# zubair-irshad/articulated-object-nerf

Hardware: AMD Instinct MI355X
Metric: rays/sec (64c+128f samples) (higher is better)
Workload: dtype f32; 1 GPU; sapien-single-scene vanilla NeRF full-frame render 640x480, 65 coarse + 193 fine evals/ray, 307200 rays per GPU per step, randomized=False, white_bkgd=True; rays_per_gpu=307200, evals_per_ray=258, exchange=none

## Files before the change

### articulated-object-nerf_amd/csrc/aon_common.h

```cpp
#pragma once

#include <hip/hip_runtime.h>
#include <stdint.h>

#include <atomic>

namespace aon {

typedef float f32x4 __attribute__((ext_vector_type(4)));
typedef float f32x16 __attribute__((ext_vector_type(16)));

#define AON_HALF_PI_F32 1.57079637050628662109375f

__device__ __forceinline__ float sin_f32(float x) {
  const float ax = __builtin_fabsf(x);
  const float k = __builtin_rintf(ax * 0.636619747f);
  const int q = (int)k;
  float r = __builtin_fmaf(k, -0x1.921fb4p+0f, ax);
  r = __builtin_fmaf(k, -0x1.4442d0p-24f, r);
  r = __builtin_fmaf(k, -0x1.846988p-48f, r);
  const float z = r * r;
  float ps = __builtin_fmaf(z, -1.9515295891e-4f, 8.3321608736e-3f);
  ps = __builtin_fmaf(z, ps, -1.6666654611e-1f);
  const float s = __builtin_fmaf(r * z, ps, r);
  float pc = __builtin_fmaf(z, 2.443315711809948e-5f, -1.388731625493765e-3f);
  pc = __builtin_fmaf(z, pc, 4.166664568298827e-2f);
  const float c = __builtin_fmaf(z * z, pc, __builtin_fmaf(z, -0.5f, 1.0f));
  float res = (q & 1) ? c : s;
  res = (q & 2) ? -res : res;
  return x < 0.f ? -res : res;
}

__device__ __forceinline__ float cos_f32(float x) {
  const float ax = __builtin_fabsf(x);
  const float k = __builtin_rintf(ax * 0.636619747f);
  const int q = (int)k;
  float r = __builtin_fmaf(k, -0x1.921fb4p+0f, ax);
  r = __builtin_fmaf(k, -0x1.4442d0p-24f, r);
  r = __builtin_fmaf(k, -0x1.846988p-48f, r);
  const float z = r * r;
  float ps = __builtin_fmaf(z, -1.9515295891e-4f, 8.3321608736e-3f);
  ps = __builtin_fmaf(z, ps, -1.6666654611e-1f);
  const float s = __builtin_fmaf(r * z, ps, r);
  float pc = __builtin_fmaf(z, 2.443315711809948e-5f, -1.388731625493765e-3f);
  pc = __builtin_fmaf(z, pc, 4.166664568298827e-2f);
  const float c = __builtin_fmaf(z * z, pc, __builtin_fmaf(z, -0.5f, 1.0f));
  float res = (q & 1) ? s : c;
  return ((q + 1) & 2) ? -res : res;
}

__device__ __forceinline__ float softplus_f32(float x) {
  const float z = __builtin_amdgcn_exp2f(__fmul_rn(__builtin_fabsf(x), -1.44269502162933349609375f));
  float p = 0.001986696617677808f;
  p = __builtin_fmaf(p, z, -0.013187826611101627f);
  p = __builtin_fmaf(p, z, 0.041006576269865036f);
  p = __builtin_fmaf(p, z, -0.08188041299581528f);
  p = __builtin_fmaf(p, z, 0.12377995997667313f);
  p = __builtin_fmaf(p, z, -0.16087622940540314f);
  p = __builtin_fmaf(p, z, 0.19885820150375366f);
  p = __builtin_fmaf(p, z, -0.24986496567726135f);
  p = __builtin_fmaf(p, z, 0.33332496881484985f);
  p = __builtin_fmaf(p, z, -0.4999997913837433f);
  p = __builtin_fmaf(p, z, 1.0f);
  return __fadd_rn(__builtin_fmaxf(x, 0.f), __fmul_rn(z, p));
}

__device__ __forceinline__ float sigmoid_f32(float x) {
  const float e = __builtin_amdgcn_exp2f(__fmul_rn(x, -1.44269502162933349609375f));
  const float d = __fadd_rn(1.0f, e);
  const float r = __builtin_amdgcn_rcpf(d);
  const float s = __builtin_fmaf(__builtin_fmaf(-d, r, 1.0f), r, r);
  return x < -87.0f ? 0.f : s;
}

__device__ __forceinline__ float torch_max(float a, float b) {
  if (a != a || b != b) return __builtin_nanf("");
  return a < b ? b : a;
}
__device__ __forceinline__ float torch_min(float a, float b) {
  if (a != a || b != b) return __builtin_nanf("");
  return b < a ? b : a;
}

constexpr int kNetWidth = 256;
constexpr int kCondWidth = 128;
constexpr int kPosEnc = 63;
constexpr int kViewEnc = 27;

constexpr int kChL0 = 0;
constexpr int kChL1 = 2;
constexpr int kChL5 = 34;
constexpr int kChL6 = 44;
constexpr int kChL7 = 52;
constexpr int kChBott = 60;
constexpr int kChView = 68;
constexpr int kNumChunks = 77;
constexpr int kNumBigChunks = 68;
constexpr int kBigChunkBytes = 8 * 4096;
constexpr int kSmallChunkBytes = 4 * 4096;

__host__ __device__ constexpr int chunk_bytes(int c) { return c < kNumBigChunks ? kBigChunkBytes : kSmallChunkBytes; }
__host__ __device__ constexpr int64_t chunk_offset(int c) {
  return c < kNumBigChunks ? (int64_t)c * kBigChunkBytes
                           : (int64_t)kNumBigChunks * kBigChunkBytes + (int64_t)(c - kNumBigChunks) * kSmallChunkBytes;
}
constexpr int64_t kStreamBytes = chunk_offset(kNumChunks);

constexpr int kChFView = 60;
constexpr int kNumChunksF = 69;
__host__ __device__ constexpr int chunk_bytes_f(int c) { return c < kChFView ? kBigChunkBytes : kSmallChunkBytes; }
__host__ __device__ constexpr int64_t chunk_offset_f(int c) {
  return c < kChFView ? (int64_t)c * kBigChunkBytes : (int64_t)kChFView * kBigChunkBytes + (int64_t)(c - kChFView) * kSmallChunkBytes;
}
constexpr int64_t kStreamBytesF = chunk_offset_f(kNumChunksF);
constexpr int64_t kFoldTmpOff = kStreamBytesF;
static_assert(kStreamBytesF + (128 * 256 + 128) * 4 <= kStreamBytes, "fold temporaries fit between the folded stream and the small block");

constexpr int kSmBias = 0;
constexpr int kSmBiasBott = 8 * 256;
constexpr int kSmBiasView = kSmBiasBott + 256;
constexpr int kSmWSigma = kSmBiasView + 128;
constexpr int kSmWRgb = kSmWSigma + 256;
constexpr int kSmBSigma = kSmWRgb + 384;
constexpr int kSmBRgb = kSmBSigma + 1;
constexpr int kSmallFloats = 3076;
constexpr int64_t kSmallBytes = kSmallFloats * 4;

constexpr int64_t kPackedBytes = kStreamBytes + kSmallBytes;

constexpr int kPlE = 0;
__host__ __device__ constexpr int plane_h(int l) { return 64 + 256 * l; }
constexpr int kPlBot = 64 + 8 * 256;
constexpr int kPlVE = kPlBot + 256;
constexpr int kPlHV = kPlVE + 32;
constexpr int kPlRows = kPlHV + 128;
constexpr int kMaskLayers = 9;

constexpr int kAPlPos = 0;
__host__ __device__ constexpr int aplane_d(int l) { return 32 + 128 * l; }
constexpr int kAPlE = 32 + 4 * 128;
__host__ __device__ constexpr int aplane_h(int l) { return kAPlE + 64 + 256 * l; }
constexpr int kAPlBot = kAPlE + 64 + 8 * 256;
constexpr int kAPlVE = kAPlBot + 256;
__host__ __device__ constexpr int aplane_v(int l) { return kAPlVE + 32 + 128 * l; }
constexpr int kAPlRows = kAPlVE + 32 + 4 * 128;
constexpr int kAMaskLayers = 16;

constexpr int kNumVanillaParams = 24;

struct ActParams {
  int act;
  float rgb_scale, rgb_shift, sigma_bias;
  const float* noise;
  float noise_std;
};
inline ActParams default_act(int act) { return ActParams{act, 1.002f, 0.001f, -1.0f, nullptr, 0.f}; }

struct ChainSeg {
  const char* packed_bwd;
  const float* small;
  const float* d_raw;
  const void* masks;
  const float* planes;
  float* dplanes;
  float* dxp;
  int64_t Np;
};

struct TrainSeg {
  const char* packed;
  const float* small;
  const float* rays_o; const float* rays_d; const float* viewdirs;
  const float* t_vals;
  int64_t n_rays; int S;
  float* raw;
  float* planes; void* masks;
  int64_t np_total;
  const float* view_bias = nullptr;
};

template <class T>
__device__ __forceinline__ T block_excl_scan(T v, T& total, T* red) {
  constexpr int kThreads = 256;
  const int lane = threadIdx.x & 63, wave = threadIdx.x >> 6;
  T x = v;
#pragma unroll
  for (int d = 1; d < 64; d <<= 1) {
    const T y = __shfl_up(x, d);
    if (lane >= d) x += y;
  }
  if (lane == 63) red[wave] = x;
  __syncthreads();
  T base = 0;
  total = 0;
#pragma unroll
  for (int w = 0; w < kThreads / 64; ++w) {
    const T t = red[w];
    if (w < wave) base += t;
    total += t;
  }
  __syncthreads();
  return base + x - v;
}

struct OccGrid {
  const uint32_t* bits;
  int64_t cells[3];
  float lo[3], step[3], hi[3];
};

constexpr int kMaxDevices = 64;

struct DeviceOnce {
  std::atomic<uint64_t> done{0};
};

template <class Kernel>
inline hipError_t set_max_lds(Kernel* kernel, int bytes, DeviceOnce& once) {
  int dev = 0;
  if (hipError_t e = hipGetDevice(&dev); e != hipSuccess) return e;
  if (dev < 0 || dev >= kMaxDevices) return hipErrorInvalidDevice;
  const uint64_t bit = 1ull << dev;
  if (once.done.load(std::memory_order_acquire) & bit) return hipSuccess;
  if (hipError_t e = hipFuncSetAttribute(reinterpret_cast<const void*>(kernel), hipFuncAttributeMaxDynamicSharedMemorySize, bytes);
      e != hipSuccess)
    return e;
  once.done.fetch_or(bit, std::memory_order_release);
  return hipSuccess;
}

}
```

### articulated-object-nerf_amd/csrc/aon_mlp.hip

```cpp
#include "aon_launch.h"
#include "aon_mlp_core.h"

namespace aon {

struct VanillaNet {
  static constexpr int kSlotBytes = kPairSlotBytes;
  static constexpr bool kPair = true;
  static constexpr int kNumChunks = aon::kNumChunks;
  static constexpr int chunk_bytes(int c) { return aon::chunk_bytes(c); }
};
struct VanillaFoldNet {
  static constexpr int kSlotBytes = kPairSlotBytes;
  static constexpr bool kPair = true;
  static constexpr int kNumChunks = aon::kNumChunksF;
  static constexpr int chunk_bytes(int c) { return aon::chunk_bytes_f(c); }
};
struct VanillaFoldVbNet {
  static constexpr int kSlotBytes = kPairSlotBytes;
  static constexpr bool kPair = true;
  static constexpr int kNumChunks = aon::kNumChunksF - 1;
  static constexpr int chunk_bytes(int c) { return aon::chunk_bytes_f(c < kChFView ? c : c + 1); }
  static constexpr int skip_before(int c) { return c == kChFView ? kSmallChunkBytes : 0; }
};

struct PackArgs {
  const float* p[kNumVanillaParams];
};

template <bool FOLD>
__global__ void pack_vanilla_kernel(PackArgs a, float* __restrict__ packed, int L, int Lv) {
  const int P = 3 + 6 * L, V = 3 + 6 * Lv;
  const int64_t idx = (int64_t)blockIdx.x * blockDim.x + threadIdx.x;
  constexpr int64_t stream_floats = kStreamBytes / 4;
  constexpr int64_t used_floats = FOLD ? kStreamBytesF / 4 : stream_floats;
  const float* Wf = packed + kFoldTmpOff / 4;
  if (idx >= stream_floats + kSmallFloats) return;
  if (idx >= used_floats && idx < stream_floats) {
    if (idx >= used_floats + 128 * 256 + 128) packed[idx] = 0.f;
    return;
  }
  if (idx >= stream_floats) {
    const int s = (int)(idx - stream_floats);
    float v = 0.f;
    if (s < kSmBiasBott) v = a.p[2 * (s >> 8) + 1][s & 255];
    else if (s < kSmBiasView) v = a.p[19][s - kSmBiasBott];
    else if (s < kSmWSigma) v = FOLD ? Wf[128 * 256 + s - kSmBiasView] : a.p[17][s - kSmBiasView];
    else if (s < kSmWRgb) v = a.p[20][s - kSmWSigma];
    else if (s < kSmBSigma) v = a.p[22][s - kSmWRgb];
    else if (s < kSmBRgb) v = a.p[21][0];
    else if (s < kSmBRgb + 3) v = a.p[23][s - kSmBRgb];
    packed[idx] = v;
    return;
  }
  int c, r, nt;
  constexpr int nbig = FOLD ? kChFView : kNumBigChunks;
  if (idx < (int64_t)nbig * (kBigChunkBytes / 4)) {
    c = (int)(idx / (kBigChunkBytes / 4)); r = (int)(idx % (kBigChunkBytes / 4)); nt = 8;
  } else {
    const int64_t i2 = idx - (int64_t)nbig * (kBigChunkBytes / 4);
    c = nbig + (int)(i2 / (kSmallChunkBytes / 4)); r = (int)(i2 % (kSmallChunkBytes / 4)); nt = 4;
    if constexpr (FOLD) c = c == kChFView ? kChView + 8 : c - 1 + (kChView - kChFView);
  }
  const int cc = r & 3, lane = (r >> 2) & 63, rest = r >> 8;
  const int tp = rest % nt, q = rest / nt;
  const int h = lane >> 5, row = 32 * tp + (lane & 31);
  const float* W; int ld, n_out = 256, col;
  const int hid_col = 8 * q + 4 * h + cc;
  auto pcol = [&](int c63) { return c63 < 0 ? -1 : pos_col_in(c63, L); };
  auto vcol = [&](int c27) { return c27 < 0 ? -1 : view_col_in(c27, Lv); };
  if (c < kChL1) { W = a.p[0]; ld = P; col = pcol(posenc_col(c, q, cc, h)); }
  else if (c < kChL5) { const int l = 1 + (c - kChL1) / 8; W = a.p[2 * l]; ld = 256; col = 32 * ((c - kChL1) % 8) + hid_col; }
  else if (c < kChL5 + 8) { W = a.p[10]; ld = 256 + P; col = 32 * (c - kChL5) + hid_col; }
  else if (c < kChL6) { W = a.p[10]; ld = 256 + P; col = pcol(posenc_col(c - kChL5 - 8, q, cc, h)); if (col >= 0) col += 256; }
  else if (c < kChL7) { W = a.p[12]; ld = 256; col = 32 * (c - kChL6) + hid_col; }
  else if (c < kChBott) { W = a.p[14]; ld = 256; col = 32 * (c - kChL7) + hid_col; }
  else if (c < kChView) { W = a.p[18]; ld = 256; col = 32 * (c - kChBott) + hid_col; }
  else if (c < kChView + 8) {
    W = a.p[16]; ld = 256 + V; n_out = kCondWidth; col = 32 * (c - kChView) + hid_col;
    if constexpr (FOLD) { W = Wf; ld = 256; }
  }
  else { W = a.p[16]; ld = 256 + V; n_out = kCondWidth; col = vcol(viewenc_col(q, cc, h)); if (col >= 0) col += 256; }
  packed[idx] = (col >= 0 && row < n_out) ? W[(int64_t)row * ld + col] : 0.f;
}

struct MlpSeg {
  const char* packed;
  const float* rays_o;
  const float* rays_d;
  const float* viewdirs;
  const float* t_vals;
  const float* samples_enc;
  const float* viewdirs_enc;
  float* raw;
  int64_t total;
  int S;
  int npass;
  union {
    float* planes;
    const int* gather_idx;
  };
  union {
    u32x4* masks;
    const int64_t* gather_count;
  };
  int64_t Np;
  const float* view_bias;
};
struct MlpArgs {
  MlpSeg seg[2];
  int npass_total;
};

constexpr int kLdsBytes = kRingBytes + (int)kSmallBytes;

template <bool ENC_IN_KERNEL, bool TRAIN, bool FOLD, bool VB = false, bool GATHER = false>
__global__ void __launch_bounds__(256) mlp_fwd_kernel(MlpArgs args) {
  static_assert(FOLD || !VB, "the per-ray view bias belongs to the folded form");
  static_assert(!GATHER || (ENC_IN_KERNEL && !TRAIN), "the occupancy list serves the inference kernel on in-kernel encodings");
  using Net = std::conditional_t<VB, VanillaFoldVbNet, std::conditional_t<FOLD, VanillaFoldNet, VanillaNet>>;
  extern __shared__ __attribute__((aligned(16))) char smem[];
  float* sm = reinterpret_cast<float*>(smem + kRingBytes);

  const int tid = threadIdx.x;
  const int lane = tid & 63, wave = tid >> 6;
  const int m = lane & 31, h = lane >> 5;
  const int wave_s = __builtin_amdgcn_readfirstlane(wave);

  const int64_t listed = GATHER ? *args.seg[0].gather_count : 0;
  const int npass0 = GATHER ? (int)((listed + 127) / 128) : args.seg[0].npass;
  int cur = (int)blockIdx.x >= npass0 ? 1 : 0;
  auto load_small = [&](const char* packed) {
    const f32x4* src = reinterpret_cast<const f32x4*>(packed + kStreamBytes);
    f32x4* dst = reinterpret_cast<f32x4*>(sm);
    for (int i = tid; i < kSmallFloats / 4; i += 256) dst[i] = src[i];
  };
  load_small(args.seg[cur].packed);

  Pipe p;
  pipe_init<Net>(p, args.seg[cur].packed, smem, wave, lane);

  for (int gpass = blockIdx.x; gpass < (GATHER ? npass0 : args.npass_total); gpass += gridDim.x) {
    const int si = gpass >= npass0 ? 1 : 0;
    if (si != cur) {
      __syncthreads();
      load_small(args.seg[si].packed);
      __syncthreads();
      cur = si;
    }
    const MlpSeg& sg = args.seg[si];
    const int pass = gpass - (si ? npass0 : 0);
    {
      const int nxt = gpass + (int)gridDim.x;
      p.stream = sg.packed;
      p.next_stream = args.seg[(nxt >= npass0 && nxt < (GATHER ? npass0 : args.npass_total)) ? 1 : si].packed;
    }
    int64_t g = (int64_t)pass * 128 + wave * 32 + m;
    bool valid;
    int64_t gc;
    if constexpr (GATHER) {
      valid = g < listed;
      g = gc = sg.gather_idx[valid ? g : listed - 1];
    } else {
      valid = g < sg.total;
      gc = valid ? g : sg.total - 1;
    }
    const int64_t ray = gc / sg.S;

    f32x16 E[2], V;
    float x[3] = {0.f, 0.f, 0.f}, vd[3] = {0.f, 0.f, 0.f};
    if constexpr (ENC_IN_KERNEL) {
      const float t = sg.t_vals[gc];
#pragma unroll
      for (int a = 0; a < 3; ++a) {
        x[a] = __fadd_rn(sg.rays_o[ray * 3 + a], __fmul_rn(t, sg.rays_d[ray * 3 + a]));
        vd[a] = sg.viewdirs[ray * 3 + a];
      }
      encode_pos(x, h, E);
      if constexpr (!VB || TRAIN) encode_view(vd, h, V);
    } else {
      load_pos_enc(sg.samples_enc + gc * kPosEnc, h, E);
      if constexpr (!VB || TRAIN) load_view_enc(sg.viewdirs_enc + ray * kViewEnc, h, V);
    }
    int ray32 = (int)ray;
    (void)ray32;

    PlaneIO io{};
    unsigned moff = 0;
    if constexpr (TRAIN) { io = make_plane_io(sg.planes, kPlRows, (int64_t)pass * 4 + wave_s, m, h); moff = mask_lane_off(pass, tid); }
    if constexpr (TRAIN) {
      store_pos_enc_plane(E, io, kPlE, h);
      store_view_enc_plane(V, io, kPlVE, h);
    }
    auto consume = [&](const f32x16 (&in)[8], int in_row, u32x4& mw, bool with_mask) {
      return [&, in_row, with_mask](int j) {
        return [&, in_row, with_mask, j](int i) {
          if constexpr (TRAIN) {
            if (i < 16) {
              if ((i & 3) == 0) store_quad<false>(io, in_row + 32 * j, i >> 2, in[j]);
              if (with_mask) mw[j >> 1] = mask_push_post(mw[j >> 1], in[j][i]);
            }
          }
        };
      };
    };
    auto put_mask = [&](const u32x4& mw, int mask_layer) {
      if constexpr (TRAIN)
        *mask_ptr(sg.masks, sg.Np, mask_layer, moff) = u32x4{mask_word_finish(mw[0]), mask_word_finish(mw[1]), mask_word_finish(mw[2]), mask_word_finish(mw[3])};
    };
    f32x16 X[8], Y[8];
    u32x4 mw;
    init_bias(X, sm + kSmBias + 0 * 256, h);
    chunk_mma<Net, kChL0 + 0, 8, 16>(p, E[0], X);
    chunk_mma<Net, kChL0 + 1, 8, 16>(p, E[1], X);
    relu_tiles(X);
    mw = u32x4{0u, 0u, 0u, 0u}; init_bias(Y, sm + kSmBias + 1 * 256, h); dense_layer<Net, kChL1 + 0, 8, 8>(p, X, Y, consume(X, plane_h(0), mw, true)); put_mask(mw, 0); relu_tiles(Y);
    mw = u32x4{0u, 0u, 0u, 0u}; init_bias(X, sm + kSmBias + 2 * 256, h); dense_layer<Net, kChL1 + 8, 8, 8>(p, Y, X, consume(Y, plane_h(1), mw, true)); put_mask(mw, 1); relu_tiles(X);
    mw = u32x4{0u, 0u, 0u, 0u}; init_bias(Y, sm + kSmBias + 3 * 256, h); dense_layer<Net, kChL1 + 16, 8, 8>(p, X, Y, consume(X, plane_h(2), mw, true)); put_mask(mw, 2); relu_tiles(Y);
    mw = u32x4{0u, 0u, 0u, 0u}; init_bias(X, sm + kSmBias + 4 * 256, h); dense_layer<Net, kChL1 + 24, 8, 8>(p, Y, X, consume(Y, plane_h(3), mw, true)); put_mask(mw, 3); relu_tiles(X);
    mw = u32x4{0u, 0u, 0u, 0u}; init_bias(Y, sm + kSmBias + 5 * 256, h);
    dense_layer<Net, kChL5, 8, 8>(p, X, Y, consume(X, plane_h(4), mw, true)); put_mask(mw, 4);
#ifdef AON_TRAIN_REENCODE
    if constexpr (TRAIN && ENC_IN_KERNEL) {
      asm volatile("" : "+v"(x[0]), "+v"(x[1]), "+v"(x[2]));
      encode_pos(x, h, E);
    }
#endif
    if constexpr (TRAIN && !ENC_IN_KERNEL) {
      int64_t gq = gc;
      asm volatile("" : "+v"(gq));
      load_pos_enc(sg.samples_enc + gq * kPosEnc, h, E);
    }
    chunk_mma<Net, kChL5 + 8, 8, 16>(p, E[0], Y);
    chunk_mma<Net, kChL5 + 9, 8, 16>(p, E[1], Y);
    relu_tiles(Y);
    mw = u32x4{0u, 0u, 0u, 0u}; init_bias(X, sm + kSmBias + 6 * 256, h); dense_layer<Net, kChL6, 8, 8>(p, Y, X, consume(Y, plane_h(5), mw, true)); put_mask(mw, 5); relu_tiles(X);
    f32x16 Z[4];
    mw = u32x4{0u, 0u, 0u, 0u}; init_bias(Y, sm + kSmBias + 7 * 256, h);
    if constexpr (VB) {
      asm volatile("" : "+v"(ray32));
      const float* vb = sg.view_bias + (int64_t)ray32 * kCondWidth + 4 * h;
      auto l7_side = [&](int j) {
        auto base = consume(X, plane_h(6), mw, true)(j);
        return [&, base, j, vb](int i) {
          base(i);
          if (j == 7 && i < 16) {
            const f32x4 v = *reinterpret_cast<const f32x4*>(vb + 32 * (i >> 2) + 8 * (i & 3));
            Z[i >> 2][4 * (i & 3)] = v[0]; Z[i >> 2][4 * (i & 3) + 1] = v[1]; Z[i >> 2][4 * (i & 3) + 2] = v[2]; Z[i >> 2][4 * (i & 3) + 3] = v[3];
          }
        };
      };
      dense_layer<Net, kChL7, 8, 8>(p, X, Y, l7_side);
    } else {
      dense_layer<Net, kChL7, 8, 8>(p, X, Y, consume(X, plane_h(6), mw, true));
    }
    put_mask(mw, 6); relu_tiles(Y);
    float sigma = head_partial<8>(Y, sm + kSmWSigma, h);
    sigma = sigma + __shfl_xor(sigma, 32) + sm[kSmBSigma];
    constexpr int kChV = FOLD ? kChFView : kChView;
    auto reencode_view = [&]() {
      if constexpr (TRAIN && ENC_IN_KERNEL) {
        asm volatile("" : "+v"(vd[0]), "+v"(vd[1]), "+v"(vd[2]));
        encode_view(vd, h, V);
      }
      if constexpr (TRAIN && !ENC_IN_KERNEL) {
        int64_t rq = ray;
        asm volatile("" : "+v"(rq));
        load_view_enc(sg.viewdirs_enc + rq * kViewEnc, h, V);
      }
    };
    if constexpr (FOLD) {
      mw = u32x4{0u, 0u, 0u, 0u};
      if constexpr (!VB) {
        init_bias(Z, sm + kSmBiasView, h);
        reencode_view();
        chunk_mma<Net, kChV, 4, 14>(p, V, Z);
      }
      dense_layer<Net, kChV + (VB ? 0 : 1), 8, 4>(p, Y, Z, consume(Y, plane_h(7), mw, true)); put_mask(mw, 7);
    } else {
      mw = u32x4{0u, 0u, 0u, 0u}; init_bias(X, sm + kSmBiasBott, h); dense_layer<Net, kChBott, 8, 8>(p, Y, X, consume(Y, plane_h(7), mw, true)); put_mask(mw, 7);
      init_bias(Z, sm + kSmBiasView, h);
      dense_layer<Net, kChV, 8, 4>(p, X, Z, consume(X, kPlBot, mw, false));
      reencode_view();
      chunk_mma<Net, kChV + 8, 4, 14>(p, V, Z);
    }
    relu_tiles(Z);
    if constexpr (TRAIN) {
      *mask_ptr(sg.masks, sg.Np, 8, moff) = relu_mask_bits(Z);
      store_plane(Z, io, kPlHV);
    }
    float rgb[3];
#pragma unroll
    for (int ch = 0; ch < 3; ++ch) {
      float v = head_partial<4>(Z, sm + kSmWRgb + ch * kCondWidth, h);
      rgb[ch] = v + __shfl_xor(v, 32) + sm[kSmBRgb + ch];
    }
    if (valid && h == 0) {
      f32x4 o; o[0] = rgb[0]; o[1] = rgb[1]; o[2] = rgb[2]; o[3] = sigma;
      reinterpret_cast<f32x4*>(sg.raw)[g] = o;
    }
  }
  asm volatile("s_waitcnt vmcnt(0)" ::: "memory");
}

void vanilla_fold_jobs_fwd(const float* const* params, float* packed, int view_levels, FoldGemm jobs[2]) {
  float* Wf = packed + kFoldTmpOff / 4;
  fold_view_jobs(params[16], 256 + 3 + 6 * view_levels, params[17], params[18], params[19], Wf, Wf + 128 * 256, jobs);
}

hipError_t launch_pack_vanilla(const float* const* params, float* packed, hipStream_t stream, int pos_levels, int view_levels, bool fold_done) {
  PackArgs a;
  for (int i = 0; i < kNumVanillaParams; ++i) a.p[i] = params[i];
  const int64_t n = kStreamBytes / 4 + kSmallFloats;
  const int form = fold_default();
  set_stream_form(packed, form);
  if (form == kFormFolded) {
    if (!fold_done) {
      FoldGemm jobs[2];
      vanilla_fold_jobs_fwd(params, packed, view_levels, jobs);
      if (hipError_t e = launch_fold_gemms(jobs, 2, stream); e != hipSuccess) return e;
    }
    pack_vanilla_kernel<true><<<dim3((unsigned)((n + 255) / 256)), dim3(256), 0, stream>>>(a, packed, pos_levels, view_levels);
  } else {
    pack_vanilla_kernel<false><<<dim3((unsigned)((n + 255) / 256)), dim3(256), 0, stream>>>(a, packed, pos_levels, view_levels);
  }
  return hipGetLastError();
}

int num_cus() {
  static std::atomic<int> cache[kMaxDevices];
  int dev = 0;
  if (hipGetDevice(&dev) != hipSuccess) return -1;
  if (dev < 0 || dev >= kMaxDevices) return -1;
  int cus = cache[dev].load(std::memory_order_relaxed);
  if (cus == 0) {
    hipDeviceProp_t prop;
    if (hipGetDeviceProperties(&prop, dev) != hipSuccess) return -1;
    cus = prop.multiProcessorCount;
    cache[dev].store(cus, std::memory_order_relaxed);
  }
  return cus;
}

template <bool ENC, bool TRAIN, bool FOLD, bool VB = false, bool GATHER = false>
static hipError_t launch_mlp_tf(const MlpArgs& args, hipStream_t stream) {
  static DeviceOnce lds_once;
  if (hipError_t e = set_max_lds(&mlp_fwd_kernel<ENC, TRAIN, FOLD, VB, GATHER>, kLdsBytes, lds_once); e != hipSuccess) return e;
  const int g_num_cus = num_cus();
  if (g_num_cus <= 0) return hipErrorInvalidDevice;
  const int grid = args.npass_total < g_num_cus ? args.npass_total : g_num_cus;
  if (grid <= 0) return hipSuccess;
  mlp_fwd_kernel<ENC, TRAIN, FOLD, VB, GATHER><<<dim3(grid), dim3(256), kLdsBytes, stream>>>(args);
  return hipGetLastError();
}

template <bool ENC, bool TRAIN, bool GATHER = false>
static hipError_t launch_mlp_t(const MlpArgs& args, hipStream_t stream) {
  const int form = stream_form(args.seg[0].packed);
  if (form == kFormUnknown) return hipErrorInvalidValue;
  if (args.seg[1].npass > 0 && stream_form(args.seg[1].packed) != form) return hipErrorInvalidValue;
  const bool vb = args.seg[0].view_bias != nullptr;
  if (args.seg[1].npass > 0 && (args.seg[1].view_bias != nullptr) != vb) return hipErrorInvalidValue;
  if (vb && form != kFormFolded) return hipErrorInvalidValue;
  if constexpr (ENC) {
    if (vb) return launch_mlp_tf<ENC, TRAIN, true, true, GATHER>(args, stream);
  } else {
    if (vb) return hipErrorInvalidValue;
  }
  return form == kFormFolded ? launch_mlp_tf<ENC, TRAIN, true, false, GATHER>(args, stream)
                             : launch_mlp_tf<ENC, TRAIN, false, false, GATHER>(args, stream);
}

__global__ __launch_bounds__(256) void view_bias_kernel(const float* chunk, const float* bias_vec, const float* viewdirs, int64_t n_rays, float* out) {
  __shared__ float enc[8][2][16];
  const int tid = threadIdx.x;
  const int64_t ray0 = (int64_t)blockIdx.x * 8;
  if (tid < 16) {
    const int64_t ray = ray0 + (tid >> 1);
    if (ray < n_rays) {
      float vd[3] = {viewdirs[ray * 3], viewdirs[ray * 3 + 1], viewdirs[ray * 3 + 2]};
      f32x16 V;
      encode_view(vd, tid & 1, V);
#pragma unroll
      for (int r = 0; r < 16; ++r) enc[tid >> 1][tid & 1][r] = V[r];
    }
  }
  const int row = tid & 127, tp = row >> 5;
  const float bias = bias_vec[row];
  float w[14][2];
#pragma unroll
  for (int r = 0; r < 14; ++r)
#pragma unroll
    for (int hh = 0; hh < 2; ++hh) w[r][hh] = chunk[((((r >> 2) * 4 + tp) * 64 + hh * 32 + (row & 31)) << 2) + (r & 3)];
  __syncthreads();
  for (int k = tid >> 7; k < 8; k += 2) {
    const int64_t ray = ray0 + k;
    if (ray >= n_rays) break;
    float acc = bias;
#pragma unroll
    for (int r = 0; r < 14; ++r) {
      acc = __builtin_fmaf(w[r][0], enc[k][0][r], acc);
      acc = __builtin_fmaf(w[r][1], enc[k][1][r], acc);
    }
    out[ray * kCondWidth + row] = acc;
  }
}

hipError_t launch_view_bias_raw(const float* chunk, const float* bias_vec, const float* viewdirs, int64_t n_rays, float* out, hipStream_t stream) {
  if (n_rays <= 0) return hipSuccess;
  view_bias_kernel<<<dim3((unsigned)((n_rays + 7) / 8)), dim3(256), 0, stream>>>(chunk, bias_vec, viewdirs, n_rays, out);
  return hipGetLastError();
}

hipError_t launch_view_bias(const char* packed, const float* viewdirs, int64_t n_rays, float* out, hipStream_t stream) {
  if (stream_form(packed) != kFormFolded) return hipErrorInvalidValue;
  return launch_view_bias_raw(reinterpret_cast<const float*>(packed + chunk_offset_f(kChFView)), reinterpret_cast<const float*>(packed + kStreamBytes) + kSmBiasView,
                              viewdirs, n_rays, out, stream);
}

hipError_t launch_mlp_fwd(const char* packed, const float* rays_o, const float* rays_d, const float* viewdirs,
                          const float* t_vals, int64_t n_rays, int S, float* raw, hipStream_t stream, const float* view_bias) {
  MlpArgs args{};
  MlpSeg& a = args.seg[0];
  a.packed = packed; a.rays_o = rays_o; a.rays_d = rays_d; a.viewdirs = viewdirs; a.t_vals = t_vals; a.view_bias = view_bias;
  a.raw = raw; a.total = n_rays * S; a.S = S; a.npass = (int)((a.total + 127) / 128);
  args.seg[1] = a; args.seg[1].npass = 0; args.npass_total = a.npass;
  return launch_mlp_t<true, false>(args, stream);
}

hipError_t launch_mlp_fwd_gather(const char* packed, const float* rays_o, const float* rays_d, const float* viewdirs, const float* t_vals,
                                 int64_t n_rays, int S, float* raw, hipStream_t stream, const float* view_bias, const int* idx, const int64_t* count,
                                 int64_t max_listed) {
  MlpArgs args{};
  MlpSeg& a = args.seg[0];
  a.packed = packed; a.rays_o = rays_o; a.rays_d = rays_d; a.viewdirs = viewdirs; a.t_vals = t_vals; a.view_bias = view_bias;
  a.raw = raw; a.total = n_rays * S; a.S = S; a.npass = (int)(((max_listed > 0 ? max_listed : a.total) + 127) / 128);
  a.gather_idx = idx; a.gather_count = count;
  args.seg[1] = a; args.seg[1].npass = 0; args.npass_total = a.npass;
  return launch_mlp_t<true, false, true>(args, stream);
}

hipError_t launch_mlp_fwd_train(const char* packed, const float* rays_o, const float* rays_d, const float* viewdirs,
                                const float* t_vals, int64_t n_rays, int S, float* raw, float* planes, void* masks,
                                hipStream_t stream, int64_t np_total, const float* view_bias) {
  const TrainSeg one{packed, nullptr, rays_o, rays_d, viewdirs, t_vals, n_rays, S, raw, planes, masks, np_total, view_bias};
  return launch_mlp_fwd_train2(&one, 1, stream);
}

hipError_t launch_mlp_fwd_train2(const TrainSeg* segs, int nsegs, hipStream_t stream) {
  if (nsegs < 1 || nsegs > 2) return hipErrorInvalidValue;
  MlpArgs args{};
  for (int i = 0; i < nsegs; ++i) {
    const TrainSeg& t = segs[i];
    MlpSeg& a = args.seg[i];
    a.packed = t.packed; a.rays_o = t.rays_o; a.rays_d = t.rays_d; a.viewdirs = t.viewdirs; a.t_vals = t.t_vals;
    a.raw = t.raw; a.total = t.n_rays * t.S; a.S = t.S; a.npass = (int)((a.total + 127) / 128);
    a.planes = t.planes; a.masks = static_cast<u32x4*>(t.masks); a.Np = t.np_total > 0 ? t.np_total : (int64_t)a.npass * 128;
    a.view_bias = t.view_bias;
    args.npass_total += a.npass;
  }
  if (nsegs == 1) { args.seg[1] = args.seg[0]; args.seg[1].npass = 0; }
  else if (args.seg[0].npass == 0) { args.seg[0] = args.seg[1]; args.seg[1].npass = 0; }
  return launch_mlp_t<true, true>(args, stream);
}

hipError_t launch_mlp_fwd_train_enc(const char* packed, const float* samples_enc, const float* viewdirs_enc, int64_t n_rays, int S, float* raw,
                                    float* planes, void* masks, hipStream_t stream, int64_t np_total) {
  MlpArgs args{};
  MlpSeg& a = args.seg[0];
  a.packed = packed; a.samples_enc = samples_enc; a.viewdirs_enc = viewdirs_enc;
  a.raw = raw; a.total = n_rays * S; a.S = S; a.npass = (int)((a.total + 127) / 128);
  a.planes = planes; a.masks = static_cast<u32x4*>(masks); a.Np = np_total > 0 ? np_total : (int64_t)a.npass * 128;
  args.seg[1] = a; args.seg[1].npass = 0; args.npass_total = a.npass;
  return launch_mlp_t<false, true>(args, stream);
}

hipError_t launch_mlp_fwd_enc(const char* packed, const float* samples_enc, const float* viewdirs_enc,
                              int64_t n_rays, int S, float* raw, hipStream_t stream) {
  MlpArgs args{};
  MlpSeg& a = args.seg[0];
  a.packed = packed; a.samples_enc = samples_enc; a.viewdirs_enc = viewdirs_enc;
  a.raw = raw; a.total = n_rays * S; a.S = S; a.npass = (int)((a.total + 127) / 128);
  args.seg[1] = a; args.seg[1].npass = 0; args.npass_total = a.npass;
  return launch_mlp_t<false, false>(args, stream);
}

struct VanillaTrunkNet {
  static constexpr int kSlotBytes = kPairSlotBytes;
  static constexpr bool kPair = true;
  static constexpr int kNumChunks = kChBott;
  static constexpr int chunk_bytes(int) { return kBigChunkBytes; }
};


__global__ void __launch_bounds__(256) density_grid_kernel(GridArgs args) {
  using Net = VanillaTrunkNet;
  extern __shared__ __attribute__((aligned(16))) char smem[];
  float* sm = reinterpret_cast<float*>(smem + kRingBytes);
  const int tid = threadIdx.x;
  const int lane = tid & 63, wave = tid >> 6;
  const int m = lane & 31, h = lane >> 5;
  {
    const f32x4* src = reinterpret_cast<const f32x4*>(args.packed + kStreamBytes);
    f32x4* dst = reinterpret_cast<f32x4*>(sm);
    for (int i = tid; i < kSmallFloats / 4; i += 256) dst[i] = src[i];
  }
  Pipe p;
  pipe_init<Net>(p, args.packed, smem, wave, lane);
  for (int pass = blockIdx.x; pass < args.npass; pass += gridDim.x) {
    const int64_t l0 = (int64_t)pass * 128 + wave * 32;
    const int64_t l = l0 + m;
    float x[3];
    grid_point(args, l < args.total ? l : args.total - 1, x);
    f32x16 E[2];
    encode_pos(x, h, E);
    f32x16 X[8], Y[8];
    init_bias(X, sm + kSmBias + 0 * 256, h);
    chunk_mma<Net, kChL0 + 0, 8, 16>(p, E[0], X);
    chunk_mma<Net, kChL0 + 1, 8, 16>(p, E[1], X);
    relu_tiles(X);
    init_bias(Y, sm + kSmBias + 1 * 256, h); dense_layer<Net, kChL1 + 0, 8, 8>(p, X, Y); relu_tiles(Y);
    init_bias(X, sm + kSmBias + 2 * 256, h); dense_layer<Net, kChL1 + 8, 8, 8>(p, Y, X); relu_tiles(X);
    init_bias(Y, sm + kSmBias + 3 * 256, h); dense_layer<Net, kChL1 + 16, 8, 8>(p, X, Y); relu_tiles(Y);
    init_bias(X, sm + kSmBias + 4 * 256, h); dense_layer<Net, kChL1 + 24, 8, 8>(p, Y, X); relu_tiles(X);
    init_bias(Y, sm + kSmBias + 5 * 256, h);
    dense_layer<Net, kChL5, 8, 8>(p, X, Y);
    chunk_mma<Net, kChL5 + 8, 8, 16>(p, E[0], Y);
    chunk_mma<Net, kChL5 + 9, 8, 16>(p, E[1], Y);
    relu_tiles(Y);
    init_bias(X, sm + kSmBias + 6 * 256, h); dense_layer<Net, kChL6, 8, 8>(p, Y, X); relu_tiles(X);
    init_bias(Y, sm + kSmBias + 7 * 256, h); dense_layer<Net, kChL7, 8, 8>(p, X, Y); relu_tiles(Y);
    float sigma = head_partial<8>(Y, sm + kSmWSigma, h);
    sigma = sigma + __shfl_xor(sigma, 32) + sm[kSmBSigma];
    grid_store(args.out, l0, args.total, lane, grid_activation(sigma, args.act));
  }
  asm volatile("s_waitcnt vmcnt(0)" ::: "memory");
}

hipError_t launch_density_grid(const char* packed, const int64_t* dims, const float* lo, const float* step, int64_t g_begin, int64_t g_end,
                               int act, float* out, hipStream_t stream) {
  if (stream_form(packed) == kFormUnknown) return hipErrorInvalidValue;
  GridArgs a{};
  a.packed = packed; a.ny = dims[1]; a.nz = dims[2]; a.g_begin = g_begin; a.total = g_end - g_begin;
  for (int i = 0; i < 3; ++i) { a.lo[i] = lo[i]; a.step[i] = step[i]; }
  a.act = act; a.out = out; a.npass = (int)((a.total + 127) / 128);
  static DeviceOnce lds_once;
  if (hipError_t e = set_max_lds(&density_grid_kernel, kLdsBytes, lds_once); e != hipSuccess) return e;
  const int cus = num_cus();
  if (cus <= 0) return hipErrorInvalidDevice;
  const int grid = a.npass < cus ? a.npass : cus;
  if (grid <= 0) return hipSuccess;
  density_grid_kernel<<<dim3(grid), dim3(256), kLdsBytes, stream>>>(a);
  return hipGetLastError();
}

}
```

Baseline: 543,000 rays/s.

## Software-pipeline next pass's input fetch and positional encoding into layer MMAs

The inference MLP kernel now prefetches the next pass's ray inputs and computes its sin/cos positional encoding in small staged steps, interleaved into the side slots of the layer-7 and bottleneck/view dense layers. This hides the encoding's ALU latency and the global loads behind matrix work. The sigma head is also accumulated incrementally during the bottleneck layer. A 32-bit ray-index computation with a multiply-shift divide replaces the 64-bit division, and the host launcher splits work into chunks so indices fit in 32 bits. The cost is higher register pressure and more complex scheduling, which may reduce occupancy.

Measured after the change: 541,800 rays/s. Within noise of the previous version (-0.2%).

```diff
diff --git a/articulated-object-nerf_amd/csrc/aon_common.h b/articulated-object-nerf_amd/csrc/aon_common.h
--- a/articulated-object-nerf_amd/csrc/aon_common.h
+++ b/articulated-object-nerf_amd/csrc/aon_common.h
@@ -12,23 +12,42 @@
 
 #define AON_HALF_PI_F32 1.57079637050628662109375f
 
-__device__ __forceinline__ float sin_f32(float x) {
-  const float ax = __builtin_fabsf(x);
-  const float k = __builtin_rintf(ax * 0.636619747f);
-  const int q = (int)k;
-  float r = __builtin_fmaf(k, -0x1.921fb4p+0f, ax);
+__device__ __forceinline__ float sin_step_k(float x) { return __builtin_rintf(__builtin_fabsf(x) * 0.636619747f); }
+__device__ __forceinline__ float sin_step_r(float x, float k) {
+  float r = __builtin_fmaf(k, -0x1.921fb4p+0f, __builtin_fabsf(x));
   r = __builtin_fmaf(k, -0x1.4442d0p-24f, r);
-  r = __builtin_fmaf(k, -0x1.846988p-48f, r);
-  const float z = r * r;
-  float ps = __builtin_fmaf(z, -1.9515295891e-4f, 8.3321608736e-3f);
-  ps = __builtin_fmaf(z, ps, -1.6666654611e-1f);
-  const float s = __builtin_fmaf(r * z, ps, r);
-  float pc = __builtin_fmaf(z, 2.443315711809948e-5f, -1.388731625493765e-3f);
-  pc = __builtin_fmaf(z, pc, 4.166664568298827e-2f);
-  const float c = __builtin_fmaf(z * z, pc, __builtin_fmaf(z, -0.5f, 1.0f));
-  float res = (q & 1) ? c : s;
+  return __builtin_fmaf(k, -0x1.846988p-48f, r);
+}
+__device__ __forceinline__ float sin_step_ps(float r, float& z) {
+  z = r * r;
+  const float ps = __builtin_fmaf(z, -1.9515295891e-4f, 8.3321608736e-3f);
+  return __builtin_fmaf(z, ps, -1.6666654611e-1f);
+}
+__device__ __forceinline__ float sin_step_s(float r, float z, float ps) { return __builtin_fmaf(r * z, ps, r); }
+__device__ __forceinline__ float sin_step_pc(float z, float& zz) {
+  const float pc = __builtin_fmaf(z, 2.443315711809948e-5f, -1.388731625493765e-3f);
+  zz = z * z;
+  return __builtin_fmaf(z, pc, 4.166664568298827e-2f);
+}
+__device__ __forceinline__ float sin_step_choose(float k, float z, float zz, float pc, float s, int& q) {
+  q = (int)k;
+  const float c = __builtin_fmaf(zz, pc, __builtin_fmaf(z, -0.5f, 1.0f));
+  return (q & 1) ? c : s;
+}
+__device__ __forceinline__ float sin_step_sign(float x, int q, float res) {
   res = (q & 2) ? -res : res;
   return x < 0.f ? -res : res;
+}
+__device__ __forceinline__ float sin_f32(float x) {
+  float z, zz;
+  int q;
+  const float k = sin_step_k(x);
+  const float r = sin_step_r(x, k);
+  const float ps = sin_step_ps(r, z);
+  const float s = sin_step_s(r, z, ps);
+  const float pc = sin_step_pc(z, zz);
+  const float res = sin_step_choose(k, z, zz, pc, s, q);
+  return sin_step_sign(x, q, res);
 }
 
 __device__ __forceinline__ float cos_f32(float x) {
diff --git a/articulated-object-nerf_amd/csrc/aon_mlp.hip b/articulated-object-nerf_amd/csrc/aon_mlp.hip
--- a/articulated-object-nerf_amd/csrc/aon_mlp.hip
+++ b/articulated-object-nerf_amd/csrc/aon_mlp.hip
@@ -113,6 +113,18 @@
 
 constexpr int kLdsBytes = kRingBytes + (int)kSmallBytes;
 
+__device__ __forceinline__ unsigned pass_lane(const MlpSeg& s, int pass, int wave_s, int m, unsigned& gc) {
+  const unsigned last = (unsigned)s.total - 1u, S = (unsigned)s.S;
+  unsigned base = (unsigned)pass * 128u + (unsigned)wave_s * 32u;
+  base = base < last ? base : last;
+  const unsigned q0 = base / S, r0 = base - q0 * S;
+  const unsigned M = 65535u / S + 1u;
+  const unsigned g = base + (unsigned)m;
+  gc = g < last ? g : last;
+  const unsigned r = r0 + (gc - base);
+  return q0 + (S > 32u ? (r >= S ? 1u : 0u) : (r * M) >> 16);
+}
+
 template <bool ENC_IN_KERNEL, bool TRAIN, bool FOLD, bool VB = false, bool GATHER = false>
 __global__ void __launch_bounds__(256) mlp_fwd_kernel(MlpArgs args) {
   static_assert(FOLD || !VB, "the per-ray view bias belongs to the folded form");
@@ -139,6 +151,32 @@
   Pipe p;
   pipe_init<Net>(p, args.seg[cur].packed, smem, wave, lane);
 
+  constexpr bool PIPE = ENC_IN_KERNEL && !TRAIN && !GATHER;
+  f32x16 E[2], V;
+  unsigned ray_nx = 0;
+  float in7[7], xn[3] = {0.f, 0.f, 0.f};
+  unsigned gc_nx = 0;
+  auto locate = [&](int gp) {
+    const int s = gp >= npass0 ? 1 : 0;
+    ray_nx = pass_lane(args.seg[s], gp - (s ? npass0 : 0), wave_s, m, gc_nx);
+  };
+  auto fetch_inputs = [&](int gp) {
+    const MlpSeg& ns = args.seg[gp >= npass0 ? 1 : 0];
+    in7[0] = ns.t_vals[gc_nx];
+#pragma unroll
+    for (int a = 0; a < 3; ++a) { in7[1 + a] = ns.rays_o[(int64_t)ray_nx * 3 + a]; in7[4 + a] = ns.rays_d[(int64_t)ray_nx * 3 + a]; }
+  };
+  auto form_x = [&]() {
+#pragma unroll
+    for (int a = 0; a < 3; ++a) xn[a] = __fadd_rn(in7[1 + a], __fmul_rn(in7[0], in7[4 + a]));
+  };
+  if constexpr (PIPE) {
+    locate((int)blockIdx.x);
+    fetch_inputs((int)blockIdx.x);
+    form_x();
+    encode_pos(xn, h, E);
+  }
+
   for (int gpass = blockIdx.x; gpass < (GATHER ? npass0 : args.npass_total); gpass += gridDim.x) {
     const int si = gpass >= npass0 ? 1 : 0;
     if (si != cur) {
@@ -164,11 +202,19 @@
       valid = g < sg.total;
       gc = valid ? g : sg.total - 1;
     }
-    const int64_t ray = gc / sg.S;
-
-    f32x16 E[2], V;
+    int64_t ray;
+    if constexpr (PIPE) ray = ray_nx; else ray = gc / sg.S;
+    const int ng = gpass + (int)gridDim.x < args.npass_total ? gpass + (int)gridDim.x : gpass;
+    (void)ng;
+
     float x[3] = {0.f, 0.f, 0.f}, vd[3] = {0.f, 0.f, 0.f};
-    if constexpr (ENC_IN_KERNEL) {
+    if constexpr (PIPE) {
+      if constexpr (!VB) {
+#pragma unroll
+        for (int a = 0; a < 3; ++a) vd[a] = sg.viewdirs[ray * 3 + a];
+        encode_view(vd, h, V);
+      }
+    } else if constexpr (ENC_IN_KERNEL) {
       const float t = sg.t_vals[gc];
 #pragma unroll
       for (int a = 0; a < 3; ++a) {
@@ -236,6 +282,68 @@
     mw = u32x4{0u, 0u, 0u, 0u}; init_bias(X, sm + kSmBias + 6 * 256, h); dense_layer<Net, kChL6, 8, 8>(p, Y, X, consume(Y, plane_h(5), mw, true)); put_mask(mw, 5); relu_tiles(X);
     f32x16 Z[4];
     mw = u32x4{0u, 0u, 0u, 0u}; init_bias(Y, sm + kSmBias + 7 * 256, h);
+    float sig_acc = 0.f;
+    f32x4 sig_w = {0.f, 0.f, 0.f, 0.f};
+    const float enc_phase = h ? AON_HALF_PI_F32 : 0.f;
+    auto sigma_slot = [&](int j, int i) {
+      if (i < 16) {
+        if ((i & 3) == 0) sig_w = *reinterpret_cast<const f32x4*>(sm + kSmWSigma + 32 * j + 8 * (i >> 2) + 4 * h);
+        sig_acc = __builtin_fmaf(sig_w[i & 3], Y[j][i], sig_acc);
+      }
+    };
+    float sx = 0.f, sk = 0.f, sr = 0.f, sz = 0.f, szz = 0.f, sps = 0.f, ss = 0.f, spc = 0.f, sres = 0.f;
+    int sq = 0;
+    auto enc_slot = [&](int u) {
+      const int rho = u >> 3, st = u & 7;
+      if (rho < 30) {
+        if (st == 0) {
+          float xr = xn[rho % 3];
+          asm volatile("" : "+v"(xr));
+          sx = __fadd_rn(__fmul_rn(xr, (float)(1 << (rho / 3))), enc_phase);
+          asm volatile("" : "+v"(sx));
+        } else if (st == 1) {
+          sk = sin_step_k(sx);
+          asm volatile("" : "+v"(sk));
+        } else if (st == 2) {
+          sr = sin_step_r(sx, sk);
+          asm volatile("" : "+v"(sr));
+        } else if (st == 3) {
+          sps = sin_step_ps(sr, sz);
+          asm volatile("" : "+v"(sps), "+v"(sz));
+        } else if (st == 4) {
+          ss = sin_step_s(sr, sz, sps);
+          asm volatile("" : "+v"(ss));
+        } else if (st == 5) {
+          spc = sin_step_pc(sz, szz);
+          asm volatile("" : "+v"(spc), "+v"(szz));
+        } else if (st == 6) {
+          sres = sin_step_choose(sk, sz, szz, spc, ss, sq);
+          asm volatile("" : "+v"(sres), "+v"(sq));
+        } else {
+          float e = sin_step_sign(sx, sq, sres);
+          asm volatile("" : "+v"(e));
+          E[rho >> 4][rho & 15] = e;
+        }
+      } else if (st == 0) {
+        float e = rho == 30 ? (h ? xn[2] : xn[0]) : (h ? 0.f : xn[1]);
+        asm volatile("" : "+v"(e));
+        E[1][rho - 16] = e;
+      }
+    };
+    auto in_slot = [&](int j, int i) {
+      if (j == 0 && i == 8) { locate(ng); asm volatile("" : "+v"(gc_nx), "+v"(ray_nx)); }
+      if (j == 0 && i == 12) fetch_inputs(ng);
+      if (j == 2 && i == 0) form_x();
+      if (j >= 4) enc_slot(32 * (j - 4) + i);
+    };
+    auto y_side = [&](int j) {
+      return [&, j](int i) {
+        sigma_slot(j, i);
+        if constexpr (FOLD) enc_slot(128 + 16 * j + i);
+      };
+    };
+    auto x_side = [&](int j) { return [&, j](int i) { enc_slot(128 + 16 * j + i); }; };
+    auto l7_pipe = [&](int j) { return [&, j](int i) { in_slot(j, i); }; };
     if constexpr (VB) {
       asm volatile("" : "+v"(ray32));
       const float* vb = sg.view_bias + (int64_t)ray32 * kCondWidth + 4 * h;
@@ -243,6 +351,7 @@
         auto base = consume(X, plane_h(6), mw, true)(j);
         return [&, base, j, vb](int i) {
           base(i);
+          if constexpr (PIPE) in_slot(j, i);
           if (j == 7 && i < 16) {
             const f32x4 v = *reinterpret_cast<const f32x4*>(vb + 32 * (i >> 2) + 8 * (i & 3));
             Z[i >> 2][4 * (i & 3)] = v[0]; Z[i >> 2][4 * (i & 3) + 1] = v[1]; Z[i >> 2][4 * (i & 3) + 2] = v[2]; Z[i >> 2][4 * (i & 3) + 3] = v[3];
@@ -250,12 +359,17 @@
         };
       };
       dense_layer<Net, kChL7, 8, 8>(p, X, Y, l7_side);
+    } else if constexpr (PIPE) {
+      dense_layer<Net, kChL7, 8, 8>(p, X, Y, l7_pipe);
     } else {
       dense_layer<Net, kChL7, 8, 8>(p, X, Y, consume(X, plane_h(6), mw, true));
     }
     put_mask(mw, 6); relu_tiles(Y);
-    float sigma = head_partial<8>(Y, sm + kSmWSigma, h);
-    sigma = sigma + __shfl_xor(sigma, 32) + sm[kSmBSigma];
+    float sigma = 0.f;
+    if constexpr (!PIPE) {
+      sigma = head_partial<8>(Y, sm + kSmWSigma, h);
+      sigma = sigma + __shfl_xor(sigma, 32) + sm[kSmBSigma];
+    }
     constexpr int kChV = FOLD ? kChFView : kChView;
     auto reencode_view = [&]() {
       if constexpr (TRAIN && ENC_IN_KERNEL) {
@@ -275,15 +389,22 @@
         reencode_view();
         chunk_mma<Net, kChV, 4, 14>(p, V, Z);
       }
-      dense_layer<Net, kChV + (VB ? 0 : 1), 8, 4>(p, Y, Z, consume(Y, plane_h(7), mw, true)); put_mask(mw, 7);
+      if constexpr (PIPE) dense_layer<Net, kChV + (VB ? 0 : 1), 8, 4>(p, Y, Z, y_side);
+      else dense_layer<Net, kChV + (VB ? 0 : 1), 8, 4>(p, Y, Z, consume(Y, plane_h(7), mw, true));
+      put_mask(mw, 7);
     } else {
-      mw = u32x4{0u, 0u, 0u, 0u}; init_bias(X, sm + kSmBiasBott, h); dense_layer<Net, kChBott, 8, 8>(p, Y, X, consume(Y, plane_h(7), mw, true)); put_mask(mw, 7);
+      mw = u32x4{0u, 0u, 0u, 0u}; init_bias(X, sm + kSmBiasBott, h);
+      if constexpr (PIPE) dense_layer<Net, kChBott, 8, 8>(p, Y, X, y_side);
+      else dense_layer<Net, kChBott, 8, 8>(p, Y, X, consume(Y, plane_h(7), mw, true));
+      put_mask(mw, 7);
       init_bias(Z, sm + kSmBiasView, h);
-      dense_layer<Net, kChV, 8, 4>(p, X, Z, consume(X, kPlBot, mw, false));
+      if constexpr (PIPE) dense_layer<Net, kChV, 8, 4>(p, X, Z, x_side);
+      else dense_layer<Net, kChV, 8, 4>(p, X, Z, consume(X, kPlBot, mw, false));
       reencode_view();
       chunk_mma<Net, kChV + 8, 4, 14>(p, V, Z);
     }
     relu_tiles(Z);
+    if constexpr (PIPE) sigma = sig_acc + __shfl_xor(sig_acc, 32) + sm[kSmBSigma];
     if constexpr (TRAIN) {
       *mask_ptr(sg.masks, sg.Np, 8, moff) = relu_mask_bits(Z);
       store_plane(Z, io, kPlHV);
@@ -292,6 +413,7 @@
 #pragma unroll
     for (int ch = 0; ch < 3; ++ch) {
       float v = head_partial<4>(Z, sm + kSmWRgb + ch * kCondWidth, h);
+      if constexpr (PIPE) asm("" : "+v"(v));
       rgb[ch] = v + __shfl_xor(v, 32) + sm[kSmBRgb + ch];
     }
     if (valid && h == 0) {
@@ -419,12 +541,22 @@
 
 hipError_t launch_mlp_fwd(const char* packed, const float* rays_o, const float* rays_d, const float* viewdirs,
                           const float* t_vals, int64_t n_rays, int S, float* raw, hipStream_t stream, const float* view_bias) {
-  MlpArgs args{};
-  MlpSeg& a = args.seg[0];
-  a.packed = packed; a.rays_o = rays_o; a.rays_d = rays_d; a.viewdirs = viewdirs; a.t_vals = t_vals; a.view_bias = view_bias;
-  a.raw = raw; a.total = n_rays * S; a.S = S; a.npass = (int)((a.total + 127) / 128);
-  args.seg[1] = a; args.seg[1].npass = 0; args.npass_total = a.npass;
-  return launch_mlp_t<true, false>(args, stream);
+  if (S <= 0) return hipErrorInvalidValue;
+  const int64_t max_rays = (((int64_t)1 << 31) - 1) / S;
+  if (max_rays == 0) return hipErrorInvalidValue;
+  int64_t r0 = 0;
+  do {
+    const int64_t n = n_rays - r0 < max_rays ? n_rays - r0 : max_rays;
+    MlpArgs args{};
+    MlpSeg& a = args.seg[0];
+    a.packed = packed; a.rays_o = rays_o + r0 * 3; a.rays_d = rays_d + r0 * 3; a.viewdirs = viewdirs ? viewdirs + r0 * 3 : nullptr;
+    a.t_vals = t_vals + r0 * S; a.view_bias = view_bias ? view_bias + r0 * kCondWidth : nullptr;
+    a.raw = raw + r0 * S * 4; a.total = n * S; a.S = S; a.npass = (int)((a.total + 127) / 128);
+    args.seg[1] = a; args.seg[1].npass = 0; args.npass_total = a.npass;
+    if (hipError_t e = launch_mlp_t<true, false>(args, stream); e != hipSuccess) return e;
+    r0 += n;
+  } while (r0 < n_rays);
+  return hipSuccess;
 }
 
 hipError_t launch_mlp_fwd_gather(const char* packed, const float* rays_o, const float* rays_d, const float* viewdirs, const float* t_vals,
```
